# Jabruson/FDN-TIP2025

Measured on AMD Instinct MI355X. Metric: images/sec, FDN (LPNet->FDN forward) 1280x720 bs=8 fp32, higher is better.
Workload: dtype f32; 1 GPU; BASELINE.json configs[1]: FDN 1280x720 (padded 1280x736) batch=8 per GPU fp32; global_batch=8, parallelism=batch-shard x1, weights=synthetic (tamed 0.03) FDN + real LPNet, hip_streams=1, rccl_ranks=1, hip_graph=True, fdsa_full=False, fdsa_pair=False, no_tail_pin=False, tail_pin_l2=False, narrow_pipe=False, unfused_mlps=False, stats_launches=False, resample_upsample=False, aff_resized=False

## Files before the change

fdn-tip2025_amd/csrc/fcaffn_in.hip:

```cpp
#include "common.hpp"

namespace {

using f32x16 = fdn_f32x16;

struct Args {
    const float *xi, *x1, *img, *w, *gamma, *beta, *w1m, *w3m, *w1a, *w3a;
    const float *stats1, *gamma1, *beta1;
    float* out;
    int B, C, H, W;
    int tiles_per_img, total_tiles;
};

constexpr int MS = 15;

template <int NCH, int VEC>
__global__ __launch_bounds__(256, 2) void fcaffn_in_kernel(Args a) {
    extern __shared__ __attribute__((aligned(16))) float smem[];
    typedef typename VecT<VEC>::type vf;
    constexpr int C = 32 * NCH, KS = 16 * NCH, NS = C + 1, NT = 256;
    const int H = a.H, W = a.W;
    const unsigned P = (unsigned)(H * W), P4 = P * 4u;
    float* tg = smem;
    float* tb = tg + C;
    float* Wl = tb + C;
    float* Wm = Wl + C * NS;
    float* Wa = Wm + 2 * MS * NS;
    float* tg1 = Wa + 2 * MS * NS;
    float* tb1 = tg1 + C;
    const bool ln1 = a.stats1 != nullptr;
    const int tid = threadIdx.x, lane = tid & 63, wave = tid >> 6, kh = lane >> 5, ln = lane & 31;
    for (int i = tid; i < C; i += NT) {
        tg[i] = a.gamma[i]; tb[i] = a.beta[i];
        tg1[i] = ln1 ? a.gamma1[i] : 1.f; tb1[i] = ln1 ? a.beta1[i] : 0.f;
    }
    for (int idx = tid; idx < C * C; idx += NT) {
        const int k = idx % C, n = idx / C;
        Wl[k * NS + n] = a.w[(long)n * C + k];
    }
    for (int idx = tid; idx < 2 * MS * C; idx += NT) {
        const int j = idx % (2 * MS), n = idx / (2 * MS), c = j / 10, t = j - c * 10;
        Wm[j * NS + n] = t < 9 ? a.w3m[n * 9 + t] * a.w1m[n * 3 + c] : 0.f;
        Wa[j * NS + n] = t < 9 ? a.w3a[n * 9 + t] * a.w1a[n * 3 + c] : 0.f;
    }
    __syncthreads();

    unsigned tapoff[5], lmask[5], rmask[5];
#pragma unroll
    for (int s5 = 0; s5 < 5; ++s5) {
        const int t = 2 * s5 + kh, dy = t / 3 - 1, dx = t % 3 - 1;
        tapoff[s5] = t < 9 ? (unsigned)((dy * W + dx) * 4) : 0x80000000u;
        lmask[s5] = (t < 9 && dx == -1) ? 0xFFFFFFFFu : 0u;
        rmask[s5] = (t < 9 && dx == 1) ? 0xFFFFFFFFu : 0u;
    }
    const float r_W = 1.0f / (float)W;

    struct Tile { int b; unsigned pix; bool ok; };
    auto tile_setup = [&](int t) {
        Tile r;
        r.b = t / a.tiles_per_img;
        const unsigned p_ = (unsigned)(t - r.b * a.tiles_per_img) * (4 * 32 * VEC) + (wave * 32 + ln) * VEC;
        r.ok = p_ < P;
        r.pix = r.ok ? p_ : P - VEC;
        return r;
    };
    vf xa[KS], xb[KS];
    vf pa[MS];
    auto strip_issue = [&](const float* base, const Tile& t, vf (&dst)[KS], int s0, int s1) __attribute__((always_inline)) {
        const rsrc_t r0 = mk_rsrc(base + (long)t.b * C * P, (unsigned)C * P4);
        const unsigned voff = (kh * P + t.pix) * 4u;
#pragma unroll
        for (int s = 0; s < KS; ++s)
            if (s >= s0 && s < s1) dst[s] = bloadv<VEC>(r0, voff, (unsigned)(2 * s) * P4);
    };
    vf mu1 = 0.f, rs1 = 0.f;
    auto stats1_issue = [&](const Tile& t) __attribute__((always_inline)) {
        if (ln1) {
            const rsrc_t r1 = mk_rsrc(a.stats1 + (long)t.b * 2 * P, 2u * P4);
            mu1 = bloadv<VEC>(r1, t.pix * 4u, 0u);
            rs1 = bloadv<VEC>(r1, t.pix * 4u, P4);
        }
    };
    auto patch_issue = [&](const Tile& t) __attribute__((always_inline)) {
#pragma unroll
        for (int s = 0; s < MS; ++s) {
            const rsrc_t rc = mk_rsrc(a.img + ((long)t.b * 3 + s / 5) * P, P4);
#pragma unroll
            for (int v = 0; v < VEC; ++v)
                pa[s][v] = __uint_as_float(__builtin_amdgcn_raw_buffer_load_b32(rc, t.pix * 4u + 4u * v + tapoff[s % 5], 0u, 0));
        }
    };

    int tile = blockIdx.x;
    bool live = tile < a.total_tiles;
    Tile cur = tile_setup(live ? tile : 0);
    if (live) {
        strip_issue(a.xi, cur, xa, 0, KS);
        strip_issue(a.x1, cur, xb, 0, KS);
        stats1_issue(cur);
        patch_issue(cur);
    }
    while (live) {
        vf sm = 0.f;
#pragma unroll
        for (int s = 0; s < KS; ++s) sm += xa[s];
        vf mean, sq = 0.f, rstd;
#pragma unroll
        for (int v = 0; v < VEC; ++v) mean[v] = (sm[v] + __shfl_xor(sm[v], 32)) / (float)C;
#pragma unroll
        for (int s = 0; s < KS; ++s) { const vf dl = xa[s] - mean; sq += dl * dl; }
#pragma unroll
        for (int v = 0; v < VEC; ++v) rstd[v] = 1.0f / sqrtf((sq[v] + __shfl_xor(sq[v], 32)) / (float)C + 1e-5f);
        if (ln1) {
#pragma unroll
            for (int s = 0; s < KS; ++s) {
                asm volatile("" ::: "memory");
                xb[s] = (xb[s] - mu1) * rs1 * tg1[2 * s + kh] + tb1[2 * s + kh];
            }
        }
#pragma unroll
        for (int s = 0; s < KS; ++s) {
            asm volatile("" ::: "memory");
            const float ga = tg[2 * s + kh], be = tb[2 * s + kh];
            xa[s] = ((xa[s] - mean) * rstd * ga + be) * xb[s] + xb[s];
        }
        {
            const unsigned y = P < (1u << 22) ? (unsigned)(((float)cur.pix + 0.5f) * r_W) : cur.pix / (unsigned)W;
            const unsigned x = cur.pix - y * (unsigned)W;
#pragma unroll
            for (int v = 0; v < VEC; ++v) {
                const unsigned lft = (x + v == 0u) ? 0xFFFFFFFFu : 0u, rgt = (x + v == (unsigned)W - 1u) ? 0xFFFFFFFFu : 0u;
#pragma unroll
                for (int s5 = 0; s5 < 5; ++s5) {
                    const unsigned keep = ~((lmask[s5] & lft) | (rmask[s5] & rgt));
#pragma unroll
                    for (int c = 0; c < 3; ++c) pa[c * 5 + s5][v] = __uint_as_float(__float_as_uint(pa[c * 5 + s5][v]) & keep);
                }
            }
        }
        const int ntile = tile + gridDim.x;
        const bool nlive = ntile < a.total_tiles;
        const Tile nxt = tile_setup(nlive ? ntile : tile);
        if (nlive) { strip_issue(a.x1, nxt, xb, 0, KS); stats1_issue(nxt); }

        const rsrc_t ro = mk_rsrc(a.out + (long)cur.b * C * P, (unsigned)C * P4);
        const unsigned voff = cur.ok ? (4u * kh * P + cur.pix) * 4u : 0x80000000u;
#pragma unroll 1
        for (int m = 0; m < NCH; ++m) {
            const bool refill = nlive && m == NCH - 1;
            f32x16 acc[VEC], am[VEC], aa[VEC];
#pragma unroll
            for (int v = 0; v < VEC; ++v)
#pragma unroll
                for (int r = 0; r < 16; ++r) { acc[v][r] = 0.f; am[v][r] = 0.f; aa[v][r] = 0.f; }
            const float* w = Wl + kh * NS + m * 32 + ln;
            float ar[2][8];
#pragma unroll
            for (int i = 0; i < 8; ++i) ar[0][i] = w[i * 2 * NS];
#pragma unroll
            for (int grp = 0; grp < KS / 8; ++grp) {
                if (grp + 1 < KS / 8) {
#pragma unroll
                    for (int i = 0; i < 8; ++i) ar[(grp + 1) & 1][i] = w[((grp + 1) * 8 + i) * 2 * NS];
                }
                __builtin_amdgcn_sched_barrier(0);
#pragma unroll
                for (int i = 0; i < 8; ++i)
#pragma unroll
                    for (int v = 0; v < VEC; ++v)
                        acc[v] = __builtin_amdgcn_mfma_f32_32x32x2f32(ar[grp & 1][i], xa[grp * 8 + i][v], acc[v], 0, 0, 0);
                if (refill) strip_issue(a.xi, nxt, xa, grp * 8, grp * 8 + 8);
            }
            const float* wm = Wm + kh * NS + m * 32 + ln;
            const float* wa = Wa + kh * NS + m * 32 + ln;
            float mr[MS], dr[MS];
#pragma unroll
            for (int s = 0; s < MS; ++s) { mr[s] = wm[s * 2 * NS]; dr[s] = wa[s * 2 * NS]; }
            __builtin_amdgcn_sched_barrier(0);
#pragma unroll
            for (int s = 0; s < MS; ++s)
#pragma unroll
                for (int v = 0; v < VEC; ++v) {
                    am[v] = __builtin_amdgcn_mfma_f32_32x32x2f32(mr[s], pa[s][v], am[v], 0, 0, 0);
                    aa[v] = __builtin_amdgcn_mfma_f32_32x32x2f32(dr[s], pa[s][v], aa[v], 0, 0, 0);
                }
            if (refill) patch_issue(nxt);
#pragma unroll
            for (int r = 0; r < 16; ++r) {
                const int nrow = m * 32 + (r & 3) + 8 * (r >> 2);
                vf o;
#pragma unroll
                for (int v = 0; v < VEC; ++v) o[v] = acc[v][r] * am[v][r] + aa[v][r];
                bstorev<VEC>(o, ro, voff, (unsigned)nrow * P4);
            }
        }
        cur = nxt; tile = ntile; live = nlive;
    }
}

template <int NCH, int VEC>
int launch_fcaffn_in(Args a, hipStream_t s) {
    constexpr int C = 32 * NCH;
    const size_t lds = (4UL * C + (size_t)C * (C + 1) + 4UL * MS * (C + 1)) * sizeof(float);
    a.tiles_per_img = cdiv((long)a.H * a.W, 4 * 32 * VEC);
    a.total_tiles = a.B * a.tiles_per_img;
    auto kern = fcaffn_in_kernel<NCH, VEC>;
    const int grid = fdn_persistent_grid(kern, 256, lds, a.total_tiles, {true, 4, 0, 0});
    if (grid < 0) return FDN_ERR_LAUNCH;
    hipLaunchKernelGGL(kern, dim3(grid), dim3(256), lds, s, a);
    return fdn_launch_status();
}

}

extern "C" int fdn_fcaffn_in(const float* xi, const float* x1, const float* stats1, const float* gamma1, const float* beta1,
                             const float* img, const float* w, const float* gamma, const float* beta, const float* w1_mul,
                             const float* w3_mul, const float* w1_add, const float* w3_add, float* out, int B, int C, int H, int W,
                             fdn_stream_t stream) {
    FDN_CHECK_ARG(!stats1 || (gamma1 && beta1 && (reinterpret_cast<uintptr_t>(stats1) & 7) == 0));
    FDN_CHECK_ARG(xi && x1 && img && w && gamma && beta && w1_mul && w3_mul && w1_add && w3_add && out);
    FDN_CHECK_ARG(B > 0 && H > 0 && W > 1 && (long)H * W < (1L << 28));
    if ((C != 32 && C != 64) || W % 2 != 0) return FDN_ERR_UNSUPPORTED;
    if (((reinterpret_cast<uintptr_t>(xi) | reinterpret_cast<uintptr_t>(x1) | reinterpret_cast<uintptr_t>(out)) & 7) != 0) return FDN_ERR_UNSUPPORTED;
    Args a = {xi, x1, img, w, gamma, beta, w1_mul, w3_mul, w1_add, w3_add, stats1, gamma1, beta1, out, B, C, H, W, 0, 0};
    hipStream_t s = static_cast<hipStream_t>(stream);
    return C == 32 ? launch_fcaffn_in<1, 2>(a, s) : launch_fcaffn_in<2, 1>(a, s);
}
```

fdn-tip2025_amd/fdn_hip/ops.py:

```python
import ctypes
import functools

import torch

from . import (ACT_NONE, EPI_MULADD, EPI_NONE, EPI_RES, PRO_LN, PRO_LN3_GATE, PRO_LN_MULADD, PRO_NONE,
               Conv1x1Desc, FdnHipError, check, lib, storage_dtype, stream)

BF16 = torch.bfloat16
ERR_UNSUPPORTED = 4


def _planes(t, what, bf16_ok=False):
    if not t.is_cuda:
        raise FdnHipError(f"{what} must live on a ROCm device (got {t.device}); the FDN path has no CPU fallback")
    if t.dtype != torch.float32 and not (bf16_ok and t.dtype == BF16):
        raise FdnHipError(f"{what} must be float32{' or bfloat16 storage' if bf16_ok else ''} (got {t.dtype})")
    assert t.dim() == 4, what
    _, C, H, W = t.shape
    st = t.stride()
    if not (st[3] == 1 and st[2] == W and st[1] == H * W) and t.numel() > 0:
        raise FdnHipError(f"{what}: channel/row/column dims must be dense (strides {st})")
    return ctypes.c_void_p(t.data_ptr()), (st[0] if t.shape[0] > 1 else C * H * W)


def _flat(t, what, bf16_ok=False):
    if t is None:
        return None
    if not t.is_cuda or not (t.dtype == torch.float32 or (bf16_ok and t.dtype == BF16)) or not t.is_contiguous():
        raise FdnHipError(f"{what} must be a contiguous float32 ROCm tensor")
    return ctypes.c_void_p(t.data_ptr())


def block_storage(C, P, hidden=None):
    if storage_dtype() != "bf16" or C > 64 or P % 4:
        return torch.float32
    if hidden is not None and (hidden < 64 or hidden < 2 * C):
        return torch.float32
    return BF16


class WeightCache:

    def __init__(self):
        self._store = {}

    def get(self, name, srcs, build):
        key = tuple(None if p is None else (p.data_ptr(), p._version, str(p.device)) for p in srcs)
        hit = self._store.get(name)
        cuda = any(p is not None and p.is_cuda for p in srcs)
        cur = torch.cuda.current_stream() if cuda else None
        if hit is None or hit[0] != key:
            with torch.no_grad():
                val = build()
            ev = None
            if cuda:
                ev = torch.cuda.Event()
                ev.record(cur)
                if hit is not None:
                    self._retire(hit)
            hit = (key, val, ev, {cur.cuda_stream} if cuda else set(), tuple(srcs))
            self._store[name] = hit
        elif cuda and cur.cuda_stream not in hit[3]:
            if not torch.cuda.is_current_stream_capturing():
                cur.wait_event(hit[2])
                hit[3].add(cur.cuda_stream)
        return hit[1]

    def versions(self):
        return tuple(h[0] for h in self._store.values())

    def __deepcopy__(self, memo):
        return WeightCache()

    def __getstate__(self):
        return {"_store": {}}

    def __setstate__(self, st):
        self._store = {}

    @staticmethod
    def _retire(hit):
        for t in (hit[1] if isinstance(hit[1], (tuple, list)) else (hit[1],)):
            if torch.is_tensor(t) and t.is_cuda:
                for sid in hit[3]:
                    t.record_stream(torch.cuda.ExternalStream(sid, device=t.device))

    def clear(self):
        for hit in self._store.values():
            self._retire(hit)
        self._store = {}


_forgotten = 0


def forget_derived(*modules):
    global _forgotten
    _forgotten += 1
    for root in modules:
        for m in root.modules():
            m.__dict__.pop("_fdn_graphed", None)
            for v in m.__dict__.values():
                if isinstance(v, WeightCache):
                    v.clear()


def fold_ln(w, bias, gamma, beta):
    with torch.no_grad():
        w2 = w.reshape(w.shape[0], -1)
        wf = (w2 * gamma.reshape(1, -1)).contiguous()
        bf = torch.mv(w2.double(), beta.double()).float()
        if bias is not None:
            bf = bf + bias
    return wf, bf.contiguous()


def conv1x1_pack(w, ln3_E=0):
    N = w.shape[0]
    K = w.numel() // N
    wpk = torch.empty(lib().fdn_conv1x1_pack_bytes(N, K, ln3_E), device=w.device, dtype=torch.uint8)
    check(lib().fdn_conv1x1_pack(_flat(w.reshape(N, K), "w"), N, K, ln3_E, ctypes.c_void_p(wpk.data_ptr()), stream()), "fdn_conv1x1_pack")
    return wpk


CONV1X1_FORMS = ("refused", "split", "split_strip", "tile", "smallk_stream_vec", "smallk_stream", "kstream_vec", "narrow_tail", "smallk_vec",
                 "smallk", "generic")
_ROUTE_FIELDS = ("status", "form", "n", "pro", "nw", "early", "xbf", "obf", "strip2", "own_stats", "bf16_pipe", "threads", "tile_px")


def conv1x1_route(d):
    desc = (ctypes.c_int * len(_ROUTE_FIELDS))()
    check(lib().fdn_conv1x1_route(ctypes.byref(d), desc, len(desc)), "fdn_conv1x1_route")
    rt = dict(zip(_ROUTE_FIELDS, desc))
    rt["form"] = CONV1X1_FORMS[rt["form"]]
    return rt


def conv1x1(xs, w, bias=None, *, out=None, act=ACT_NONE, ln=None, ln3_gate=None, ln_muladd=None, res=None,
            muladd=None, want_stats=False, cache=None, out_dtype=torch.float32, route_only=False):
    if torch.is_tensor(xs):
        xs = [xs]
    B, _, H, W = xs[0].shape
    P = H * W
    N = w.shape[0]
    K = sum(x.shape[1] for x in xs)
    assert w.numel() == N * K, (w.shape, K)
    if out is None:
        out = torch.empty((B, N, H, W), device=xs[0].device, dtype=out_dtype)
    d = Conv1x1Desc()
    for i, x in enumerate(xs):
        d.x[i], d.xbs[i] = _planes(x, f"x[{i}]", bf16_ok=(i == 0 and len(xs) == 1))
        d.kseg[i] = x.shape[1]
    d.x_bf16 = int(xs[0].dtype == BF16)
    d.out_bf16 = int(out.dtype == BF16)
    d.w = _flat(w, "w")
    d.bias = _flat(bias, "bias")
    d.out, d.obs = _planes(out, "out", bf16_ok=True)
    d.B, d.K, d.N, d.P = B, K, N, P
    d.pro, d.ln_group = PRO_NONE, K
    w0, bias0 = w, bias
    if ln is not None:
        d.pro = PRO_LN
        if cache is not None:
            w, bias = cache[0].get(cache[1], [w, bias, ln[1], ln[2]], lambda w=w, bias=bias: fold_ln(w, bias, ln[1], ln[2]))
        else:
            w, bias = fold_ln(w, bias, ln[1], ln[2])
        d.w, d.bias = _flat(w, "w"), _flat(bias, "bias")
        d.stats = _flat(ln[0], "stats")
    elif ln3_gate is not None:
        d.pro, d.ln_group = PRO_LN3_GATE, K // 3
        d.stats, d.gamma, d.beta = _flat(ln3_gate[0], "stats"), _flat(ln3_gate[1], "gamma"), _flat(ln3_gate[2], "beta")
        d.xb, d.xbbs = _planes(ln3_gate[3], "v_value")
    elif ln_muladd is not None:
        d.pro = PRO_LN_MULADD
        d.stats, d.gamma, d.beta = _flat(ln_muladd[0], "stats"), _flat(ln_muladd[1], "gamma"), _flat(ln_muladd[2], "beta")
        d.xb, d.xbbs = _planes(ln_muladd[3], "x1")
    d.act = act
    d.epi = EPI_NONE
    if res is not None:
        d.epi = EPI_RES
        d.res, d.rbs = _planes(res, "res")
    elif muladd is not None:
        d.epi = EPI_MULADD
        d.mul, d.mbs = _planes(muladd[0], "mul")
        d.add, mbs2 = _planes(muladd[1], "add")
        assert mbs2 == d.mbs
    stats = None
    if want_stats and N <= 160:
        stats = torch.empty((B, 1, 2, P), device=out.device, dtype=torch.float32)
        d.stats_out = _flat(stats, "stats_out")
    rt, own_stats = None, False
    if cache is not None:
        d.wpk = ctypes.c_void_p(16)
        rt = conv1x1_route(d)
        d.wpk = None
        if rt["form"] in ("split", "split_strip"):
            srcs = [w0, bias0] + (list(ln[1:3]) if ln is not None else [])
            d.wpk = ctypes.c_void_p(cache[0].get(cache[1] + ":pk", srcs, lambda w=w: conv1x1_pack(
                w, K // 3 if ln3_gate is not None else 0)).data_ptr())
            own_stats = rt["own_stats"]
    need_stats = d.pro in (PRO_LN3_GATE, PRO_LN_MULADD) and not d.stats and not own_stats
    if route_only:
        if need_stats:
            d.stats = ctypes.c_void_p(16)
        return rt if d.wpk else conv1x1_route(d)
    if need_stats:
        auto = chan_stats(xs[0], groups=3) if ln3_gate is not None else chan_stats(xs[0])
        d.stats = _flat(auto, "stats")
    check(lib().fdn_conv1x1(ctypes.byref(d), stream()), "fdn_conv1x1")
    if want_stats:
        out._fdn_stats = stats if stats is not None else chan_stats(out)
    return out


GEMM_OWN_STATS = True


def stats_of(x):
    st = getattr(x, "_fdn_stats", None)
    return st if st is not None else chan_stats(x)


def chan_stats(x, groups=1):
    B, C, H, W = x.shape
    E = C // groups
    ptr, xbs = _planes(x, "x")
    stats = torch.empty((B, groups, 2, H * W), device=x.device, dtype=torch.float32)
    check(lib().fdn_chan_stats(ptr, ctypes.c_long(xbs), _flat(stats, "stats"), B, groups, E, H * W, stream()),
          "fdn_chan_stats")
    return stats


def layernorm_chan(x, gamma, beta):
    B, C, H, W = x.shape
    out = torch.empty_like(x)
    check(lib().fdn_layernorm_chan(_flat(x, "x"), _flat(gamma, "gamma"), _flat(beta, "beta"), _flat(out, "out"),
                                   B, C, H * W, stream()), "fdn_layernorm_chan")
    return out


def fdsa_core(hidden, dw_w, fft_w):
    B, C4, H, W = hidden.shape
    out = torch.empty_like(hidden)
    check(lib().fdn_fdsa_core(_flat(hidden, "hidden"), _flat(dw_w, "dw_w"), _flat(fft_w, "fft_w"), _flat(out, "out"),
                              B, C4 // 4, H, W, stream()), "fdn_fdsa_core")
    return out


FDSA_FUSED_C = (24, 32, 48, 64)


def fdsa_pack(w, gamma, beta):
    E4, C = w.shape[0], w.shape[1]
    E = E4 // 4
    nch = (E + 7) // 8
    wpk = torch.empty((nch, 3 * ((C + 15) // 16) + 1, 64, 4), device=w.device, dtype=torch.float32)
    check(lib().fdn_fdsa_pack(_flat(w.reshape(E4, C), "w"), _flat(gamma, "gamma"), _flat(beta, "beta"), _flat(wpk, "wpk"),
                              C, E, stream()), "fdn_fdsa_pack")
    return wpk


def fdsa_fused(x, stats, wpk, dw_w, fft_w, out_dtype=torch.float32):
    B, C, H, W = x.shape
    E = fft_w.shape[0]
    assert C in FDSA_FUSED_C, C
    out = torch.empty((B, 4 * E, H, W), device=x.device, dtype=out_dtype)
    ptr, xbs = _planes(x, "x")
    check(lib().fdn_fdsa_fused(ptr, ctypes.c_long(xbs), _flat(stats, "stats"), _flat(wpk, "wpk"), _flat(dw_w, "dw_w"),
                               _flat(fft_w, "fft_w"), _flat(out, "out", True), B, C, E, H, W, int(out_dtype == BF16), stream()),
          "fdn_fdsa_fused")
    return out


FDSA_TAIL = True
_fdsa_scratch = {}


def fdsa_tail_pack(w_out, gamma3, beta3, C, pin=None):
    N = w_out.shape[0]
    E = w_out.numel() // N // 3
    Hd = pin[0].shape[0] if pin is not None else 0
    n = lib().fdn_fdsa_tail_pack_floats(C, E, N, Hd)
    if n <= 0:
        return None
    img = torch.empty(n, device=w_out.device, dtype=torch.float32)
    check(lib().fdn_fdsa_tail_pack(_flat(w_out.reshape(N, 3 * E), "w_out"), _flat(gamma3, "gamma3"), _flat(beta3, "beta3"),
                                   _flat(pin[0].reshape(Hd, C), "pin_w") if pin is not None else None, _flat(pin[1], "pin_b") if pin is not None else None,
                                   _flat(img, "img"), C, E, N, Hd, stream()), "fdn_fdsa_tail_pack")
    return img


def fdsa_fused_tail(x, stats, wpk, dw_w, fft_w, tail_img, res=None, want_stats=False, Hd=0, h_dtype=torch.float32):
    B, C, H, W = x.shape
    E = dw_w.shape[0] // 4
    ptr, xbs = _planes(x, "x")
    n = lib().fdn_fdsa_scratch_floats(B, E, H, W)
    key = (str(x.device), n)
    scr = _fdsa_scratch.get(key)
    if scr is None:
        scr = _fdsa_scratch[key] = torch.zeros(n, device=x.device, dtype=torch.float32)
    out = torch.empty((B, C, H, W), device=x.device, dtype=torch.float32)
    st = torch.empty((B, 1, 2, H * W), device=x.device, dtype=torch.float32) if want_stats else None
    h = torch.empty((B, Hd, H, W), device=x.device, dtype=h_dtype) if Hd else None
    rc = lib().fdn_fdsa_fused_tail(ptr, ctypes.c_long(xbs), _flat(stats, "stats"), _flat(wpk, "wpk"), _flat(dw_w, "dw_w"), _flat(fft_w, "fft_w"),
                                   _flat(tail_img, "tail_img"), _flat(res, "res"), _flat(out, "out"), _flat(st, "stats_out"), _flat(scr, "scratch"),
                                   _flat(h, "h_out", True), B, C, E, H, W, Hd, int(h_dtype == BF16), stream())
    if rc == ERR_UNSUPPORTED:
        return None
    check(rc, "fdn_fdsa_fused_tail")
    if want_stats:
        out._fdn_stats = st
    if Hd:
        out._fdn_pin = h
    return out


FDSA_TAIL_PIN_MAX_C = 32
FDSA_TAIL_PIN = True
FDSA_FULL = False
FDSA_FULL_MAX_C = 32


def fdsa_full_pack(w_hidden, gamma, beta, w_out, gamma3, beta3):
    E4, C = w_hidden.shape[0], w_hidden.shape[1]
    E = E4 // 4
    nbytes = lib().fdn_fdsa_full_pack_bytes(C, E)
    if nbytes <= 0:
        return None
    wpk = torch.empty(nbytes, device=w_hidden.device, dtype=torch.uint8)
    check(lib().fdn_fdsa_full_pack(_flat(w_hidden.reshape(E4, C), "w_hidden"), _flat(gamma, "gamma"), _flat(beta, "beta"),
                                   _flat(w_out.reshape(w_out.shape[0], 3 * E), "w_out"), _flat(gamma3, "gamma3"), _flat(beta3, "beta3"),
                                   ctypes.c_void_p(wpk.data_ptr()), C, E, stream()), "fdn_fdsa_full_pack")
    return wpk


def fdsa_full(x, stats, wpk, dw_w, fft_w, res=None, want_stats=False):
    B, C, H, W = x.shape
    E = fft_w.shape[0]
    out = torch.empty((B, C, H, W), device=x.device, dtype=torch.float32)
    st = torch.empty((B, 1, 2, H * W), device=x.device, dtype=torch.float32) if want_stats else None
    ptr, xbs = _planes(x, "x")
    rc = lib().fdn_fdsa_full(ptr, ctypes.c_long(xbs), _flat(stats, "stats"), ctypes.c_void_p(wpk.data_ptr()), _flat(dw_w, "dw_w"),
                             _flat(fft_w, "fft_w"), _flat(res, "res"), _flat(out, "out"), _flat(st, "stats_out"), B, C, E, H, W, stream())
    if rc == ERR_UNSUPPORTED:
        return None
    check(rc, "fdn_fdsa_full")
    if want_stats:
        out._fdn_stats = st
    return out


def fdsa_out(o, w, gamma3, beta3, res=None, want_stats=False):
    B, C4, H, W = o.shape
    E, N, P = C4 // 4, w.shape[0], H * W
    if E > 76 or N > 64:
        return None
    out = torch.empty((B, N, H, W), device=o.device, dtype=torch.float32)
    stats = torch.empty((B, 1, 2, P), device=o.device, dtype=torch.float32) if want_stats else None
    rc = lib().fdn_fdsa_out(_flat(o, "o", True), _flat(w, "w"), _flat(gamma3, "gamma3"), _flat(beta3, "beta3"), _flat(res, "res"),
                            _flat(out, "out"), _flat(stats, "stats_out"), B, E, N, P, int(o.dtype == BF16), stream())
    if rc == ERR_UNSUPPORTED and o.dtype != BF16:
        return None
    check(rc, "fdn_fdsa_out")
    if want_stats:
        out._fdn_stats = stats
    return out


def fdffn_mid(x, w0, w2, ffta, fftp, out_dtype=None):
    B, Hd, H, W = x.shape
    out = torch.empty(x.shape, device=x.device, dtype=out_dtype or x.dtype)
    check(lib().fdn_fdffn_mid(_flat(x, "x", True), _flat(w0, "w0"), _flat(w2, "w2"), _flat(ffta, "ffta"), _flat(fftp, "fftp"),
                              _flat(out, "out", True), B, Hd, H, W, int(x.dtype == BF16), int(out.dtype == BF16), stream()),
          "fdn_fdffn_mid")
    return out


FFN_TAIL_MODE = None


def ffn_tail(y, dw_w, w, res=None, want_stats=False, mode=None, cache=None):
    B, C, H, W = y.shape
    N = w.shape[0]
    mode = mode or FFN_TAIL_MODE
    if mode is None:
        mode = "sw" if (W % 4 == 0 and N <= 64) else "split"
    if mode == "split":
        g = dwconv_gate(y, dw_w)
        return conv1x1(g, w, res=res, want_stats=want_stats, cache=cache)
    out = torch.empty((B, N, H, W), device=y.device, dtype=torch.float32)
    stats = torch.empty((B, 1, 2, H * W), device=y.device, dtype=torch.float32) if want_stats else None
    check(lib().fdn_ffn_tail(_flat(y, "y", True), _flat(dw_w, "dw_w"), _flat(w, "w"), _flat(res, "res"), _flat(out, "out"),
                             _flat(stats, "stats_out"), B, C, N, H, W, int(y.dtype == BF16), 1 if mode == "sw" else 0, stream()),
          "fdn_ffn_tail")
    if want_stats:
        out._fdn_stats = stats
    return out


def dwconv_gate(x, w, out_dtype=None):
    B, C, H, W = x.shape
    out = torch.empty(x.shape, device=x.device, dtype=out_dtype or x.dtype)
    check(lib().fdn_dwconv_gate(_flat(x, "x", True), _flat(w, "w"), _flat(out, "out", True), B, C, H, W, int(x.dtype == BF16),
                                int(out.dtype == BF16), stream()), "fdn_dwconv_gate")
    return out


def dwconv3x3(x, w, act=ACT_NONE):
    B, C, H, W = x.shape
    out = torch.empty_like(x)
    check(lib().fdn_dwconv3x3(_flat(x, "x"), _flat(w, "w"), _flat(out, "out"), B, C, H, W, act, stream()), "fdn_dwconv3x3")
    return out


def img_mod_maps(img, w1_mul, w3_mul, w1_add, w3_add):
    B, _, H, W = img.shape
    C = w1_mul.shape[0]
    mul = torch.empty((B, C, H, W), device=img.device, dtype=torch.float32)
    add = torch.empty_like(mul)
    check(lib().fdn_img_mod_maps(_flat(img, "img"), _flat(w1_mul, "w1_mul"), _flat(w3_mul, "w3_mul"),
                                 _flat(w1_add, "w1_add"), _flat(w3_add, "w3_add"), _flat(mul, "mul"), _flat(add, "add"),
                                 B, C, H, W, stream()), "fdn_img_mod_maps")
    return mul, add


FCAFFN_IN_C = (32, 64)


def fcaffn_in(xi, x1, img, w, gamma, beta, w1_mul, w3_mul, w1_add, w3_add, x1_ln=None):
    B, C, H, W = xi.shape
    out = torch.empty_like(xi)
    st1, g1, b1 = x1_ln if x1_ln is not None else (None, None, None)
    check(lib().fdn_fcaffn_in(_flat(xi, "xi"), _flat(x1, "x1"), _flat(st1, "stats1"), _flat(g1, "gamma1"), _flat(b1, "beta1"),
                              _flat(img, "img"), _flat(w, "w"), _flat(gamma, "gamma"),
                              _flat(beta, "beta"), _flat(w1_mul, "w1_mul"), _flat(w3_mul, "w3_mul"), _flat(w1_add, "w1_add"),
                              _flat(w3_add, "w3_add"), _flat(out, "out"), B, C, H, W, stream()), "fdn_fcaffn_in")
    return out


FCAFFN_PACKED_MIN_C = 96


def fcaffn_in_pack(w, w1_mul, w3_mul, w1_add, w3_add):
    C = w.shape[0]
    wpk = torch.empty(lib().fdn_fcaffn_in_pack_bytes(C), device=w.device, dtype=torch.uint8)
    check(lib().fdn_fcaffn_in_pack(_flat(w.reshape(C, C), "w"), _flat(w1_mul, "w1_mul"), _flat(w3_mul, "w3_mul"), _flat(w1_add, "w1_add"),
                                   _flat(w3_add, "w3_add"), C, ctypes.c_void_p(wpk.data_ptr()), stream()), "fdn_fcaffn_in_pack")
    return wpk


def fcaffn_in_packed(xi, stats_xi, x1, img, wpk, gamma, beta, x1_ln=None):
    B, C, H, W = xi.shape
    out = torch.empty_like(xi)
    st1, g1, b1 = x1_ln if x1_ln is not None else (None, None, None)
    check(lib().fdn_fcaffn_in_packed(_flat(xi, "xi"), _flat(stats_xi, "stats_xi"), _flat(x1, "x1"), _flat(st1, "stats1"), _flat(g1, "gamma1"),
                                     _flat(b1, "beta1"), _flat(img, "img"), ctypes.c_void_p(wpk.data_ptr()), _flat(gamma, "gamma"),
                                     _flat(beta, "beta"), _flat(out, "out"), B, C, H, W, stream()), "fdn_fcaffn_in_packed")
    return out


RS_BILINEAR_HALF, RS_BILINEAR_X2, RS_NEAREST_HALF, RS_NEAREST_X2, RS_PIXEL_UNSHUFFLE = 0, 1, 2, 3, 4


def spec_pitch(Wf):
    return (Wf + 15) // 16 * 16


FFT_ROUTES = ("refused", "planned", "inplace", "pingpong", "rader")
FFT_MAX_STAGES = 16
FFT_ROWS, FFT_IROWS, FFT_COLS = 0, 1, 2


def fft_route(kind, n):
    desc = (ctypes.c_int * (5 + 2 * FFT_MAX_STAGES))()
    check(lib().fdn_fft_route(int(kind), int(n), desc, len(desc)), "fdn_fft_route")
    nst = desc[4]
    radices = tuple(desc[5 + i] for i in range(nst))
    return {"route": FFT_ROUTES[desc[0]], "big": desc[1], "width": desc[2], "rader": desc[3], "radices": radices,
            "gather": tuple(r for i, r in enumerate(radices) if desc[5 + FFT_MAX_STAGES + i])}


def rfft_rows(x, pitch=None):
    W = x.shape[-1]
    rows = x.numel() // W
    out = torch.empty(x.shape[:-1] + (pitch or W // 2 + 1, 2), device=x.device, dtype=torch.float32)
    check(lib().fdn_rfft_rows(_flat(x, "x"), _flat(out, "out"), ctypes.c_long(rows), W, ctypes.c_long(pitch or 0), stream()), "fdn_rfft_rows")
    return out


@functools.lru_cache(maxsize=None)
def _rows_planned(W):
    return W >= 2 and W % 2 == 0 and fft_route(FFT_ROWS, W)["route"] == "planned"


def rows_ln_ok(x):
    B, _, H, W = x.shape
    return _rows_planned(W) and B * 2 * H * W * 4 <= 0x7FFFFFFF


def rfft_rows_ln(x, stats, gamma, beta, pitch=None):
    B, C, H, W = x.shape
    out = torch.empty((B, C, H, pitch or W // 2 + 1, 2), device=x.device, dtype=torch.float32)
    check(lib().fdn_rfft_rows_ln(_flat(x, "x"), _flat(stats, "stats"), _flat(gamma, "gamma"), _flat(beta, "beta"), _flat(out, "out"),
                                 B, C, H, W, ctypes.c_long(pitch or 0), stream()), "fdn_rfft_rows_ln")
    return out


def irfft_rows(z, H, W, scale, res=None, alpha=0.0, out=None):
    B, C, Hin, Wfin, _ = z.shape
    if out is None:
        out = torch.empty((B, C, H, W), device=z.device, dtype=torch.float32)
    check(lib().fdn_irfft_rows(_flat(z, "z"), ctypes.c_long(Wfin), ctypes.c_long(Hin * Wfin), _flat(out, "out"),
                               ctypes.c_long(B * C), H, W, ctypes.c_float(scale), _flat(res, "res"),
                               ctypes.c_float(alpha), stream()), "fdn_irfft_rows")
    return out


def sincos(x):
    sn, cs = torch.empty_like(x), torch.empty_like(x)
    check(lib().fdn_sincos_f32(_flat(x, "x"), _flat(sn, "sn"), _flat(cs, "cs"), ctypes.c_long(x.numel()), stream()), "fdn_sincos_f32")
    return sn, cs


def pack_guidance(amp, pha, pitch=None):
    B, _, H, Wf = amp.shape
    pitch = pitch or Wf
    cached = getattr(amp, "_fdn_packed", None)
    if cached is not None and cached[0] is pha and cached[1].shape[2] == pitch:
        return cached[1]
    out = torch.empty((B, H, pitch, 8), device=amp.device, dtype=torch.float32)
    check(lib().fdn_pack_guidance(_flat(amp, "amp"), _flat(pha, "pha"), _flat(out, "packed"), B, H, Wf, ctypes.c_long(pitch), stream()),
          "fdn_pack_guidance")
    amp._fdn_packed = (pha, out)
    return out


def fft_cols_fcaffn(z, amp, pha, wxa, wxp):
    B, C, H, Wf, _ = z.shape
    guide = pack_guidance(amp, pha, pitch=Wf)
    check(lib().fdn_fft_cols_fcaffn(_flat(z, "z"), _flat(guide, "guide"), _flat(wxa, "wxa"), _flat(wxp, "wxp"), B, C, H, Wf,
                                    stream()), "fdn_fft_cols_fcaffn")
    return z


def fft_cols_fwd(z, want_abs, want_ang, rd_before=False, fix_real=True):
    B, C, H, Wf, _ = z.shape
    oa = torch.empty((B, C, H, Wf), device=z.device, dtype=torch.float32) if want_abs else None
    og = torch.empty((B, C, H, Wf), device=z.device, dtype=torch.float32) if want_ang else None
    check(lib().fdn_fft_cols_fwd(_flat(z, "z"), _flat(oa, "abs"), _flat(og, "ang"), ctypes.c_long(B * C), H, Wf,
                                 int(rd_before), int(fix_real), stream()), "fdn_fft_cols_fwd")
    return oa, og


def fft_cols_inv_polar(mag, pha, H, Wf):
    B, C, Hin, Wfin = mag.shape
    z = torch.empty((B, C, H, Wf, 2), device=mag.device, dtype=torch.float32)
    check(lib().fdn_fft_cols_inv_polar(_flat(mag, "mag"), _flat(pha, "pha"), Hin, Wfin, _flat(z, "z"),
                                       ctypes.c_long(B * C), H, Wf, stream()), "fdn_fft_cols_inv_polar")
    return z


def conv2d(x, w, bias=None, stride=1, pad=0, act=ACT_NONE, res=None, res_before_act=False, post_add=0.0):
    B, Cin, H, W = x.shape
    Cout, _, KH, KW = w.shape
    OH, OW = (H + 2 * pad - KH) // stride + 1, (W + 2 * pad - KW) // stride + 1
    out = torch.empty((B, Cout, OH, OW), device=x.device, dtype=torch.float32)
    check(lib().fdn_conv2d(_flat(x, "x"), _flat(w, "w"), _flat(bias, "bias"), _flat(res, "res"), _flat(out, "out"),
                           B, Cin, H, W, Cout, KH, KW, stride, pad, act, int(res_before_act), ctypes.c_float(post_add),
                           stream()), "fdn_conv2d")
    return out


def maxpool2d(x, k, s):
    B, C, H, W = x.shape
    if H < k or W < k:
        raise FdnHipError(f"maxpool2d: {H}x{W} is smaller than the {k}x{k} window")
    out = torch.empty((B, C, (H - k) // s + 1, (W - k) // s + 1), device=x.device, dtype=torch.float32)
    check(lib().fdn_maxpool2d(_flat(x, "x"), _flat(out, "out"), ctypes.c_long(B * C), H, W, k, s, stream()), "fdn_maxpool2d")
    return out


def conv_transpose4x4s2(x, w, bias, act):
    B, Cin, H, W = x.shape
    Cout = w.shape[1]
    out = torch.empty((B, Cout, 2 * H, 2 * W), device=x.device, dtype=torch.float32)
    check(lib().fdn_conv_transpose4x4s2(_flat(x, "x"), _flat(w, "w"), _flat(bias, "bias"), _flat(out, "out"),
                                        B, Cin, H, W, Cout, act, stream()), "fdn_conv_transpose4x4s2")
    return out


AFF_MULTIRES = True
UPCONV_GATHER = True


def upsample_conv3x3(x, w, cache=None):
    B, C, h, w_ = x.shape
    Cout = w.shape[0]
    build = lambda: w.detach().permute(2, 3, 0, 1).reshape(9 * Cout, C).contiguous()
    wr = cache[0].get(cache[1] + ":taps", [w], build) if cache is not None else build()
    z = conv1x1(x, wr, cache=None if cache is None else (cache[0], cache[1] + ":z"))
    out = torch.empty((B, Cout, 2 * h, 2 * w_), device=x.device, dtype=torch.float32)
    check(lib().fdn_upconv_gather(_flat(z, "z"), _flat(out, "out"), B, Cout, h, w_, stream()), "fdn_upconv_gather")
    return out


def resample(x, mode, r=1):
    B, C, H, W = x.shape
    if mode in (RS_BILINEAR_HALF, RS_NEAREST_HALF):
        shp = (B, C, H // 2, W // 2)
    elif mode in (RS_BILINEAR_X2, RS_NEAREST_X2):
        shp = (B, C, 2 * H, 2 * W)
    else:
        shp = (B, C * r * r, H // r, W // r)
    out = torch.empty(shp, device=x.device, dtype=torch.float32)
    check(lib().fdn_resample(_flat(x, "x"), _flat(out, "out"), ctypes.c_long(B * C), H, W, mode, r, stream()),
          "fdn_resample")
    return out


def dw1x1_pad1(x, w, bias):
    B, C, H, W = x.shape
    out = torch.empty((B, C, H + 2, W + 2), device=x.device, dtype=torch.float32)
    check(lib().fdn_dw1x1_pad1(_flat(x, "x"), _flat(w, "w"), _flat(bias, "bias"), _flat(out, "out"), B, C, H, W,
                               stream()), "fdn_dw1x1_pad1")
    return out


def avgpool3s2(x):
    B, C, H, W = x.shape
    out = torch.empty((B, C, (H - 1) // 2 + 1, (W - 1) // 2 + 1), device=x.device, dtype=torch.float32)
    check(lib().fdn_avgpool3s2(_flat(x, "x"), _flat(out, "out"), ctypes.c_long(B * C), H, W, stream()), "fdn_avgpool3s2")
    return out


def global_avgpool(x):
    B, C, H, W = x.shape
    out = torch.empty((B, C, 1, 1), device=x.device, dtype=torch.float32)
    check(lib().fdn_global_avgpool(_flat(x, "x"), _flat(out, "out"), ctypes.c_long(B * C), ctypes.c_long(H * W),
                                   stream()), "fdn_global_avgpool")
    return out


def se_apply(y, gate, shortcut):
    B, C, H, W = y.shape
    out = torch.empty_like(y)
    check(lib().fdn_se_apply(_flat(y, "y"), _flat(gate, "gate"), _flat(shortcut, "shortcut"), _flat(out, "out"),
                             ctypes.c_long(B * C), ctypes.c_long(H * W), stream()), "fdn_se_apply")
    return out


def scale_batch_(x, ratio):
    B = x.shape[0]
    check(lib().fdn_scale_batch(_flat(x, "x"), _flat(ratio, "ratio"), B, ctypes.c_long(x.numel() // B), stream()),
          "fdn_scale_batch")
    return x


SPECTRAL_MLP_C = (12, 24)
SPECTRAL_MLP_FUSED = True


def spectral_mlp2(mag, pha, w1m, b1m, w2m, b2m, w1p, b1p, w2p, b2p, slope=0.1):
    B, C = mag.shape[0], mag.shape[1]
    P = mag[0, 0].numel()
    check(lib().fdn_spectral_mlp2(_flat(mag, "mag"), _flat(pha, "pha"), _flat(w1m.reshape(C, C), "w1m"), _flat(b1m, "b1m"), _flat(w2m.reshape(C, C), "w2m"),
                                  _flat(b2m, "b2m"), _flat(w1p.reshape(C, C), "w1p"), _flat(b1p, "b1p"), _flat(w2p.reshape(C, C), "w2p"), _flat(b2p, "b2p"),
                                  B, C, ctypes.c_long(P), ctypes.c_float(slope), stream()), "fdn_spectral_mlp2")
    return mag, pha


def gamma_curve(x, i_map, scale=40.0):
    out = torch.empty_like(x)
    check(lib().fdn_gamma_curve(_flat(x, "x"), _flat(i_map, "i_map"), _flat(out, "out"), ctypes.c_float(scale),
                                ctypes.c_long(x.numel()), stream()), "fdn_gamma_curve")
    return out
```

Measured before the change: 29.06 images/s.

## Switch fcaffn_in MFMA to bf16x3 split with pre-packed LDS weight fragments

Replaces the fp32 32x32x2 MFMA chain in the fused LN/1x1-conv/image-modulation kernel with a 3-way bf16 split emulation (split6 MFMA) on packed 8-wide K fragments. Weights are pre-split into bf16 parts in LDS, and activations and patches are cut into bf16 parts in registers. The aim is to use the higher-throughput bf16 matrix pipe while keeping near-fp32 accuracy. It also reorders the xi prefetch and adds an fp32-pipe fallback to unfused ops. The cost is extra split/pack ALU work and higher register pressure.

```diff
diff --git a/fdn-tip2025_amd/csrc/fcaffn_in.hip b/fdn-tip2025_amd/csrc/fcaffn_in.hip
--- a/fdn-tip2025_amd/csrc/fcaffn_in.hip
+++ b/fdn-tip2025_amd/csrc/fcaffn_in.hip
@@ -13,45 +13,71 @@
 };
 
 constexpr int MS = 15;
+constexpr int QM = 2;
 
 template <int NCH, int VEC>
 __global__ __launch_bounds__(256, 2) void fcaffn_in_kernel(Args a) {
     extern __shared__ __attribute__((aligned(16))) float smem[];
     typedef typename VecT<VEC>::type vf;
-    constexpr int C = 32 * NCH, KS = 16 * NCH, NS = C + 1, NT = 256;
+    constexpr int C = 32 * NCH, KS = 16 * NCH, QL = 2 * NCH, NT = 256;
     const int H = a.H, W = a.W;
     const unsigned P = (unsigned)(H * W), P4 = P * 4u;
     float* tg = smem;
     float* tb = tg + C;
-    float* Wl = tb + C;
-    float* Wm = Wl + C * NS;
-    float* Wa = Wm + 2 * MS * NS;
-    float* tg1 = Wa + 2 * MS * NS;
+    float* tg1 = tb + C;
     float* tb1 = tg1 + C;
+    fdn_u32x4* Bl = reinterpret_cast<fdn_u32x4*>(tb1 + C);
+    fdn_u32x4* Bm = Bl + NCH * QL * 3 * 64;
+    fdn_u32x4* Ba = Bm + NCH * QM * 3 * 64;
     const bool ln1 = a.stats1 != nullptr;
     const int tid = threadIdx.x, lane = tid & 63, wave = tid >> 6, kh = lane >> 5, ln = lane & 31;
     for (int i = tid; i < C; i += NT) {
         tg[i] = a.gamma[i]; tb[i] = a.beta[i];
         tg1[i] = ln1 ? a.gamma1[i] : 1.f; tb1[i] = ln1 ? a.beta1[i] : 0.f;
     }
-    for (int idx = tid; idx < C * C; idx += NT) {
-        const int k = idx % C, n = idx / C;
-        Wl[k * NS + n] = a.w[(long)n * C + k];
-    }
-    for (int idx = tid; idx < 2 * MS * C; idx += NT) {
-        const int j = idx % (2 * MS), n = idx / (2 * MS), c = j / 10, t = j - c * 10;
-        Wm[j * NS + n] = t < 9 ? a.w3m[n * 9 + t] * a.w1m[n * 3 + c] : 0.f;
-        Wa[j * NS + n] = t < 9 ? a.w3a[n * 9 + t] * a.w1a[n * 3 + c] : 0.f;
+    auto cut = [](fdn_u32x4 (&dst)[3], const float (&f)[8]) __attribute__((always_inline)) {
+        unsigned p[3][4];
+#pragma unroll
+        for (int i = 0; i < 4; ++i) fdn_split3(f[2 * i], f[2 * i + 1], p[0][i], p[1][i], p[2][i]);
+#pragma unroll
+        for (int part = 0; part < 3; ++part) dst[part] = fdn_u32x4{p[part][0], p[part][1], p[part][2], p[part][3]};
+    };
+    for (int idx = tid; idx < NCH * QL * 64; idx += NT) {
+        const int l = idx & 63, mq = idx >> 6, q = mq % QL, n = (mq / QL) * 32 + (l & 31);
+        const float* wr = a.w + (long)n * C + 16 * q + (l >> 5);
+        float f[8];
+#pragma unroll
+        for (int j = 0; j < 8; ++j) f[j] = wr[2 * j];
+        fdn_u32x4 p[3];
+        cut(p, f);
+#pragma unroll
+        for (int part = 0; part < 3; ++part) Bl[(mq * 3 + part) * 64 + l] = p[part];
+    }
+    for (int idx = tid; idx < NCH * QM * 64; idx += NT) {
+        const int l = idx & 63, mq = idx >> 6, q = mq % QM, n = (mq / QM) * 32 + (l & 31);
+        float fm[8], fa[8];
+#pragma unroll
+        for (int j = 0; j < 8; ++j) {
+            const int s = 8 * q + j, c = s / 5, t = 2 * (s % 5) + (l >> 5);
+            const bool tap = s < MS && t < 9;
+            fm[j] = tap ? a.w3m[n * 9 + t] * a.w1m[n * 3 + c] : 0.f;
+            fa[j] = tap ? a.w3a[n * 9 + t] * a.w1a[n * 3 + c] : 0.f;
+        }
+        fdn_u32x4 pm[3], pd[3];
+        cut(pm, fm);
+        cut(pd, fa);
+#pragma unroll
+        for (int part = 0; part < 3; ++part) { Bm[(mq * 3 + part) * 64 + l] = pm[part]; Ba[(mq * 3 + part) * 64 + l] = pd[part]; }
     }
     __syncthreads();
 
-    unsigned tapoff[5], lmask[5], rmask[5];
+    unsigned tapoff[5], lbits = 0u, rbits = 0u;
 #pragma unroll
     for (int s5 = 0; s5 < 5; ++s5) {
         const int t = 2 * s5 + kh, dy = t / 3 - 1, dx = t % 3 - 1;
         tapoff[s5] = t < 9 ? (unsigned)((dy * W + dx) * 4) : 0x80000000u;
-        lmask[s5] = (t < 9 && dx == -1) ? 0xFFFFFFFFu : 0u;
-        rmask[s5] = (t < 9 && dx == 1) ? 0xFFFFFFFFu : 0u;
+        lbits |= (t < 9 && dx == -1) ? 1u << s5 : 0u;
+        rbits |= (t < 9 && dx == 1) ? 1u << s5 : 0u;
     }
     const float r_W = 1.0f / (float)W;
 
@@ -66,12 +92,11 @@
     };
     vf xa[KS], xb[KS];
     vf pa[MS];
-    auto strip_issue = [&](const float* base, const Tile& t, vf (&dst)[KS], int s0, int s1) __attribute__((always_inline)) {
+    auto strip_issue = [&](const float* base, const Tile& t, vf (&dst)[KS]) __attribute__((always_inline)) {
         const rsrc_t r0 = mk_rsrc(base + (long)t.b * C * P, (unsigned)C * P4);
         const unsigned voff = (kh * P + t.pix) * 4u;
 #pragma unroll
-        for (int s = 0; s < KS; ++s)
-            if (s >= s0 && s < s1) dst[s] = bloadv<VEC>(r0, voff, (unsigned)(2 * s) * P4);
+        for (int s = 0; s < KS; ++s) dst[s] = bloadv<VEC>(r0, voff, (unsigned)(2 * s) * P4);
     };
     vf mu1 = 0.f, rs1 = 0.f;
     auto stats1_issue = [&](const Tile& t) __attribute__((always_inline)) {
@@ -95,8 +120,8 @@
     bool live = tile < a.total_tiles;
     Tile cur = tile_setup(live ? tile : 0);
     if (live) {
-        strip_issue(a.xi, cur, xa, 0, KS);
-        strip_issue(a.x1, cur, xb, 0, KS);
+        strip_issue(a.xi, cur, xa);
+        strip_issue(a.x1, cur, xb);
         stats1_issue(cur);
         patch_issue(cur);
     }
@@ -129,10 +154,10 @@
             const unsigned x = cur.pix - y * (unsigned)W;
 #pragma unroll
             for (int v = 0; v < VEC; ++v) {
-                const unsigned lft = (x + v == 0u) ? 0xFFFFFFFFu : 0u, rgt = (x + v == (unsigned)W - 1u) ? 0xFFFFFFFFu : 0u;
+                const unsigned drop = ((x + v == 0u) ? lbits : 0u) | ((x + v == (unsigned)W - 1u) ? rbits : 0u);
 #pragma unroll
                 for (int s5 = 0; s5 < 5; ++s5) {
-                    const unsigned keep = ~((lmask[s5] & lft) | (rmask[s5] & rgt));
+                    const unsigned keep = ((drop >> s5) & 1u) - 1u;
 #pragma unroll
                     for (int c = 0; c < 3; ++c) pa[c * 5 + s5][v] = __uint_as_float(__float_as_uint(pa[c * 5 + s5][v]) & keep);
                 }
@@ -141,56 +166,79 @@
         const int ntile = tile + gridDim.x;
         const bool nlive = ntile < a.total_tiles;
         const Tile nxt = tile_setup(nlive ? ntile : tile);
-        if (nlive) { strip_issue(a.x1, nxt, xb, 0, KS); stats1_issue(nxt); }
+        if (nlive) { strip_issue(a.x1, nxt, xb); stats1_issue(nxt); }
+
+        constexpr bool XI_EARLY = VEC == 1;
+        fdn_u32x4 xs[QL][VEC][3], ps[QM][VEC][3];
+        auto cut_patch = [&]() __attribute__((always_inline)) {
+#pragma unroll
+            for (int q = 0; q < QM; ++q)
+#pragma unroll
+                for (int v = 0; v < VEC; ++v) {
+                    float f[8];
+#pragma unroll
+                    for (int j = 0; j < 8; ++j) f[j] = 8 * q + j < MS ? pa[8 * q + j < MS ? 8 * q + j : 0][v] : 0.f;
+                    cut(ps[q][v], f);
+                }
+        };
+#pragma unroll
+        for (int q = 0; q < QL; ++q)
+#pragma unroll
+            for (int v = 0; v < VEC; ++v) {
+                float f[8];
+#pragma unroll
+                for (int j = 0; j < 8; ++j) f[j] = xa[8 * q + j][v];
+                cut(xs[q][v], f);
+            }
+        if (XI_EARLY && nlive) strip_issue(a.xi, nxt, xa);
+        if (NCH > 1) cut_patch();
+        __builtin_amdgcn_sched_barrier(0);
 
         const rsrc_t ro = mk_rsrc(a.out + (long)cur.b * C * P, (unsigned)C * P4);
         const unsigned voff = cur.ok ? (4u * kh * P + cur.pix) * 4u : 0x80000000u;
 #pragma unroll 1
         for (int m = 0; m < NCH; ++m) {
             const bool refill = nlive && m == NCH - 1;
-            f32x16 acc[VEC], am[VEC], aa[VEC];
+            f32x16 acc[VEC];
 #pragma unroll
             for (int v = 0; v < VEC; ++v)
 #pragma unroll
-                for (int r = 0; r < 16; ++r) { acc[v][r] = 0.f; am[v][r] = 0.f; aa[v][r] = 0.f; }
-            const float* w = Wl + kh * NS + m * 32 + ln;
-            float ar[2][8];
-#pragma unroll
-            for (int i = 0; i < 8; ++i) ar[0][i] = w[i * 2 * NS];
-#pragma unroll
-            for (int grp = 0; grp < KS / 8; ++grp) {
-                if (grp + 1 < KS / 8) {
-#pragma unroll
-                    for (int i = 0; i < 8; ++i) ar[(grp + 1) & 1][i] = w[((grp + 1) * 8 + i) * 2 * NS];
+                for (int r = 0; r < 16; ++r) acc[v][r] = 0.f;
+            const fdn_u32x4* bl = Bl + m * QL * 3 * 64 + lane;
+#pragma unroll
+            for (int q = 0; q < QL; ++q) {
+                const fdn_u32x4 wq[3] = {bl[(q * 3 + 0) * 64], bl[(q * 3 + 1) * 64], bl[(q * 3 + 2) * 64]};
+#pragma unroll
+                for (int v = 0; v < VEC; ++v) acc[v] = fdn_mfma_split6(wq, xs[q][v], acc[v]);
+            }
+            __builtin_amdgcn_sched_barrier(0);
+            if (!XI_EARLY && refill) strip_issue(a.xi, nxt, xa);
+            if (NCH == 1) cut_patch();
+            const fdn_u32x4* bm = Bm + m * QM * 3 * 64 + lane;
+            const fdn_u32x4* ba = Ba + m * QM * 3 * 64 + lane;
+#pragma unroll
+            for (int v = 0; v < VEC; ++v) {
+                f32x16 am, aa;
+#pragma unroll
+                for (int r = 0; r < 16; ++r) { am[r] = 0.f; aa[r] = 0.f; }
+#pragma unroll
+                for (int q = 0; q < QM; ++q) {
+                    const fdn_u32x4 mq[3] = {bm[(q * 3 + 0) * 64], bm[(q * 3 + 1) * 64], bm[(q * 3 + 2) * 64]};
+                    const fdn_u32x4 dq[3] = {ba[(q * 3 + 0) * 64], ba[(q * 3 + 1) * 64], ba[(q * 3 + 2) * 64]};
+                    am = fdn_mfma_split6(mq, ps[q][v], am);
+                    aa = fdn_mfma_split6(dq, ps[q][v], aa);
                 }
+#pragma unroll
+                for (int r = 0; r < 16; ++r) acc[v][r] = acc[v][r] * am[r] + aa[r];
                 __builtin_amdgcn_sched_barrier(0);
-#pragma unroll
-                for (int i = 0; i < 8; ++i)
-#pragma unroll
-                    for (int v = 0; v < VEC; ++v)
-                        acc[v] = __builtin_amdgcn_mfma_f32_32x32x2f32(ar[grp & 1][i], xa[grp * 8 + i][v], acc[v], 0, 0, 0);
-                if (refill) strip_issue(a.xi, nxt, xa, grp * 8, grp * 8 + 8);
-            }
-            const float* wm = Wm + kh * NS + m * 32 + ln;
-            const float* wa = Wa + kh * NS + m * 32 + ln;
-            float mr[MS], dr[MS];
-#pragma unroll
-            for (int s = 0; s < MS; ++s) { mr[s] = wm[s * 2 * NS]; dr[s] = wa[s * 2 * NS]; }
-            __builtin_amdgcn_sched_barrier(0);
-#pragma unroll
-            for (int s = 0; s < MS; ++s)
-#pragma unroll
-                for (int v = 0; v < VEC; ++v) {
-                    am[v] = __builtin_amdgcn_mfma_f32_32x32x2f32(mr[s], pa[s][v], am[v], 0, 0, 0);
-                    aa[v] = __builtin_amdgcn_mfma_f32_32x32x2f32(dr[s], pa[s][v], aa[v], 0, 0, 0);
-                }
+            }
             if (refill) patch_issue(nxt);
 #pragma unroll
             for (int r = 0; r < 16; ++r) {
                 const int nrow = m * 32 + (r & 3) + 8 * (r >> 2);
                 vf o;
 #pragma unroll
-                for (int v = 0; v < VEC; ++v) o[v] = acc[v][r] * am[v][r] + aa[v][r];
+                for (int v = 0; v < VEC; ++v) o[v] = acc[v][r];
                 bstorev<VEC>(o, ro, voff, (unsigned)nrow * P4);
             }
         }
@@ -201,12 +249,13 @@
 template <int NCH, int VEC>
 int launch_fcaffn_in(Args a, hipStream_t s) {
     constexpr int C = 32 * NCH;
-    const size_t lds = (4UL * C + (size_t)C * (C + 1) + 4UL * MS * (C + 1)) * sizeof(float);
+    const size_t lds = 4UL * C * sizeof(float) + (size_t)NCH * (2 * NCH + 2 * QM) * 3 * 64 * 16;
     a.tiles_per_img = cdiv((long)a.H * a.W, 4 * 32 * VEC);
     a.total_tiles = a.B * a.tiles_per_img;
     auto kern = fcaffn_in_kernel<NCH, VEC>;
     const int grid = fdn_persistent_grid(kern, 256, lds, a.total_tiles, {true, 4, 0, 0});
     if (grid < 0) return FDN_ERR_LAUNCH;
+    fdn_note_bf16_launch();
     hipLaunchKernelGGL(kern, dim3(grid), dim3(256), lds, s, a);
     return fdn_launch_status();
 }
@@ -222,6 +271,7 @@
     FDN_CHECK_ARG(B > 0 && H > 0 && W > 1 && (long)H * W < (1L << 28));
     if ((C != 32 && C != 64) || W % 2 != 0) return FDN_ERR_UNSUPPORTED;
     if (((reinterpret_cast<uintptr_t>(xi) | reinterpret_cast<uintptr_t>(x1) | reinterpret_cast<uintptr_t>(out)) & 7) != 0) return FDN_ERR_UNSUPPORTED;
+    if (fdn_matrix_pipe_f32()) return FDN_ERR_UNSUPPORTED;
     Args a = {xi, x1, img, w, gamma, beta, w1_mul, w3_mul, w1_add, w3_add, stats1, gamma1, beta1, out, B, C, H, W, 0, 0};
     hipStream_t s = static_cast<hipStream_t>(stream);
     return C == 32 ? launch_fcaffn_in<1, 2>(a, s) : launch_fcaffn_in<2, 1>(a, s);
diff --git a/fdn-tip2025_amd/fdn_hip/ops.py b/fdn-tip2025_amd/fdn_hip/ops.py
--- a/fdn-tip2025_amd/fdn_hip/ops.py
+++ b/fdn-tip2025_amd/fdn_hip/ops.py
@@ -428,13 +428,20 @@
 
 
 def fcaffn_in(xi, x1, img, w, gamma, beta, w1_mul, w3_mul, w1_add, w3_add, x1_ln=None):
+    from . import matrix_pipe
     B, C, H, W = xi.shape
     out = torch.empty_like(xi)
     st1, g1, b1 = x1_ln if x1_ln is not None else (None, None, None)
-    check(lib().fdn_fcaffn_in(_flat(xi, "xi"), _flat(x1, "x1"), _flat(st1, "stats1"), _flat(g1, "gamma1"), _flat(b1, "beta1"),
-                              _flat(img, "img"), _flat(w, "w"), _flat(gamma, "gamma"),
-                              _flat(beta, "beta"), _flat(w1_mul, "w1_mul"), _flat(w3_mul, "w3_mul"), _flat(w1_add, "w1_add"),
-                              _flat(w3_add, "w3_add"), _flat(out, "out"), B, C, H, W, stream()), "fdn_fcaffn_in")
+    rc = lib().fdn_fcaffn_in(_flat(xi, "xi"), _flat(x1, "x1"), _flat(st1, "stats1"), _flat(g1, "gamma1"), _flat(b1, "beta1"),
+                             _flat(img, "img"), _flat(w, "w"), _flat(gamma, "gamma"),
+                             _flat(beta, "beta"), _flat(w1_mul, "w1_mul"), _flat(w3_mul, "w3_mul"), _flat(w1_add, "w1_add"),
+                             _flat(w3_add, "w3_add"), _flat(out, "out"), B, C, H, W, stream())
+    if rc == ERR_UNSUPPORTED and matrix_pipe() == "f32" and C in FCAFFN_IN_C and W % 2 == 0:
+        if x1_ln is not None:
+            x1 = layernorm_chan(x1, g1, b1)
+        mul, add = img_mod_maps(img, w1_mul, w3_mul, w1_add, w3_add)
+        return conv1x1(xi, w, ln_muladd=(chan_stats(xi), gamma, beta, x1), muladd=(mul, add))
+    check(rc, "fdn_fcaffn_in")
     return out
 
 
```

Result: no change. 29.10 images/s, median of 5 (+0.1%).
